# abcouwer-jpl/zsc

Measured on AMD Instinct MI355X. Metric: deflate level-6 uncompressed MB/s in, Canterbury-like x4096 per GPU, higher is better.
Workload: dtype u8

## Files before the change

__graft_entry__.py:

```python
from __future__ import annotations

import os
import subprocess
import sys

ROOT = os.path.dirname(os.path.abspath(__file__))
if ROOT not in sys.path:
    sys.path.insert(0, ROOT)


def build() -> None:
    subprocess.run(["make", "-s", "-C", os.path.join(ROOT, "zsc_amd", "csrc")], check=True)
    subprocess.run(["make", "-s", "-C", os.path.join(ROOT, "oracle"), "oracle", "ref"], check=True)
    subprocess.run(["make", "-s", "-C", os.path.join(ROOT, "tests", "emu")], check=True)
    subprocess.run(["make", "-s", "-C", os.path.join(ROOT, "tests", "emu_sections")], check=True)
    subprocess.run(["make", "-s", "-C", os.path.join(ROOT, "tests", "emu_chunks")], check=True)
    subprocess.run(["make", "-s", "-C", os.path.join(ROOT, "tests", "emu_resync")], check=True)
    subprocess.run(["make", "-s", "-C", os.path.join(ROOT, "tests", "c_caller")], check=True)
    import zsc_amd


def smoke() -> None:
    import zsc_amd
    from zsc_amd import corpus
    from oracle.oracle_py import Oracle

    print("device:", zsc_amd.device_info())
    oracle = Oracle()
    bufs = [corpus.make_buffer(kind, size, 7 + i) for i, (kind, size) in enumerate(
        [("text", 70000), ("bitmap", 40000), ("table", 20000), ("random", 5000), ("zero", 3000),
         ("token", 257), ("text", 0)])]
    rc, outs, stats = zsc_amd.compress_batch(bufs, level=6)
# ... 18 lines not shown
```

include/zsc_hip.h:

```cpp
#ifndef ZSC_HIP_H
#define ZSC_HIP_H

#include <stdint.h>

#include "zsc/zlib_types_pub.h"

#ifdef __cplusplus
extern "C" {
#endif


I32 zsc_hip_init(I32 device_ordinal);

const char *zsc_hip_device_info(void);

void zsc_hip_release_cached_memory(void);


ZlibReturn zsc_hip_compress_batch(U32 count, const U8 *const *sources, const U32 *source_lens,
                                  U8 *const *dests, U32 *dest_lens, I32 *statuses, I32 level,
                                  I32 window_bits, I32 mem_level, ZlibStrategy strategy);

ZlibReturn zsc_hip_store_batch(U32 count, const U8 *const *sources, const U32 *source_lens,
                               const U32 *max_block_lens, U8 *const *dests, U32 *dest_lens,
// ... 32 lines not shown

ZlibReturn zsc_hip_deflate_plan_run(zsc_hip_deflate_plan *plan, const void *d_input,
                                    void *d_output, void *hip_stream);

ZlibReturn zsc_hip_deflate_plan_results(zsc_hip_deflate_plan *plan, U32 *dest_lens,
                                        I32 *statuses);

#define ZSC_HIP_NKERNELS 9
void zsc_hip_deflate_plan_profile(zsc_hip_deflate_plan *plan, I32 enable);
ZlibReturn zsc_hip_deflate_plan_times(zsc_hip_deflate_plan *plan, float *ms_out);

uint64_t zsc_hip_deflate_plan_scratch_bytes(const zsc_hip_deflate_plan *plan);

U32 zsc_hip_deflate_plan_sub_batches(const zsc_hip_deflate_plan *plan);

void zsc_hip_deflate_plan_destroy(zsc_hip_deflate_plan *plan);


typedef struct zsc_hip_inflate_plan zsc_hip_inflate_plan;

ZlibReturn zsc_hip_inflate_plan_create(zsc_hip_inflate_plan **plan, U32 count,
                                       const U32 *source_lens, const uint64_t *src_offsets,
                                       const U32 *dest_caps, const uint64_t *dst_offsets,
                                       I32 window_bits);
ZlibReturn zsc_hip_inflate_plan_create_ordered(zsc_hip_inflate_plan **plan, U32 count,
                                               const U32 *source_lens, const uint64_t *src_offsets,
                                               const U32 *dest_caps, const uint64_t *dst_offsets,
                                               I32 window_bits, const U32 *decode_order);
ZlibReturn zsc_hip_inflate_plan_run(zsc_hip_inflate_plan *plan, const void *d_src, void *d_dst,
                                    void *hip_stream);
// ... 37 lines not shown
```

zsc_amd/api.py:

```python
from __future__ import annotations

import ctypes as C
import os
import subprocess
from typing import List, Optional, Sequence, Tuple

Z_OK, Z_STREAM_END, Z_NEED_DICT = 0, 1, 2
Z_ERRNO, Z_STREAM_ERROR, Z_DATA_ERROR, Z_MEM_ERROR, Z_BUF_ERROR, Z_VERSION_ERROR = -1, -2, -3, -4, -5, -6
Z_DEFAULT_STRATEGY, Z_FILTERED, Z_HUFFMAN_ONLY, Z_RLE, Z_FIXED = 0, 1, 2, 3, 4
GZIP_CODE, DEF_WBITS, DEF_MEM_LEVEL = 16, 15, 8
NKERNELS = 9
KERNEL_NAMES = ("checksum", "hash_sort", "match_table", "parse", "parse_short", "huff_plan", "layout", "emit", "total")

_HERE = os.path.dirname(os.path.abspath(__file__))
lib_path = os.environ.get("ZSC_HIP_LIB") or os.path.join(_HERE, "libzsc_hip.so")


def build_library() -> None:
    subprocess.run(["make", "-s", "-C", os.path.join(_HERE, "csrc")], check=True)


def _load() -> C.CDLL:
    try:
        import torch
# ... 50 lines not shown
    L.zsc_hip_inflate_plan_destroy.argtypes = [C.c_void_p]
    L.zsc_hip_inflate_plan_destroy.restype = None
    L.zsc_hip_deflate_plan_layout.argtypes = [C.c_uint32, u32p, C.c_int32, C.c_int32, C.c_int32,
                                              u64p, u64p, u32p, u64p, u64p]
    L.zsc_hip_deflate_plan_create.argtypes = [C.POINTER(C.c_void_p), C.c_uint32, u32p, u64p, u64p,
                                              u32p, C.c_int32, C.c_int32, C.c_int32, C.c_int32]
    L.zsc_hip_deflate_plan_run.argtypes = [C.c_void_p, C.c_void_p, C.c_void_p, C.c_void_p]
    L.zsc_hip_deflate_plan_results.argtypes = [C.c_void_p, u32p, i32p]
    L.zsc_hip_deflate_plan_profile.argtypes = [C.c_void_p, C.c_int32]
    L.zsc_hip_deflate_plan_profile.restype = None
    L.zsc_hip_deflate_plan_times.argtypes = [C.c_void_p, C.POINTER(C.c_float)]
    L.zsc_hip_deflate_plan_scratch_bytes.argtypes = [C.c_void_p]
    L.zsc_hip_deflate_plan_scratch_bytes.restype = C.c_uint64
    L.zsc_hip_deflate_plan_sub_batches.argtypes = [C.c_void_p]
    L.zsc_hip_deflate_plan_sub_batches.restype = C.c_uint32
    L.zsc_hip_deflate_plan_destroy.argtypes = [C.c_void_p]
    L.zsc_hip_deflate_plan_destroy.restype = None
    return L


lib = _load()


def device_info() -> str:
    return lib.zsc_hip_device_info().decode()



def compress_get_min_work_buf_size(window_bits: int = DEF_WBITS, mem_level: int = DEF_MEM_LEVEL):
    out = C.c_uint32()
# ... 324 lines not shown
        self.out_caps = list(self._caps)
        self._h = C.c_void_p()
        rc = lib.zsc_hip_deflate_plan_create(C.byref(self._h), n, lens, self._in_off, self._out_off,
                                             self._caps, level, window_bits, mem_level, strategy)
        if rc != Z_OK:
            raise RuntimeError(f"zsc_hip_deflate_plan_create failed: {rc}")

    @property
    def scratch_bytes(self) -> int:
        return lib.zsc_hip_deflate_plan_scratch_bytes(self._h)

    @property
    def sub_batches(self) -> int:
        return lib.zsc_hip_deflate_plan_sub_batches(self._h)

    def profile(self, enable: bool = True) -> None:
        lib.zsc_hip_deflate_plan_profile(self._h, 1 if enable else 0)

    def run(self, d_input: int, d_output: int, stream: int = 0) -> None:
        rc = lib.zsc_hip_deflate_plan_run(self._h, C.c_void_p(d_input), C.c_void_p(d_output),
                                          C.c_void_p(stream))
        if rc != Z_OK:
            raise RuntimeError(f"zsc_hip_deflate_plan_run failed: {rc}")

    def results(self) -> Tuple[List[int], List[int]]:
        lens = (C.c_uint32 * self.count)()
        stat = (C.c_int32 * self.count)()
        rc = lib.zsc_hip_deflate_plan_results(self._h, lens, stat)
        if rc != Z_OK:
            raise RuntimeError(f"zsc_hip_deflate_plan_results failed: {rc}")
# ... 20 lines not shown
```

zsc_amd/csrc/lz_parse.h:

```cpp
#ifndef ZSC_LZ_PARSE_H
#define ZSC_LZ_PARSE_H

#include "wave.h"
#include "zsc_dev.h"

#define LZ_PR 512u
#define LZ_MIRROR 512u
#define LZ_PR_FAST 128u

template <uint32_t RING_BYTES, uint32_t CHUNK_BYTES, bool WITH_HOLES = false>
struct LzLdsT {
    static constexpr uint32_t RING = RING_BYTES, CHUNK = CHUNK_BYTES;
    static constexpr bool HAS_INS = WITH_HOLES;
    static constexpr bool HOLES = WITH_HOLES;
    static constexpr bool GLOBAL_WIN = false;
    static constexpr uint32_t PR = LZ_PR;
    uint8_t ring[RING + 512];
    uint32_t stage[WAVE];
    uint16_t prank[LZ_PR];
    uint16_t phib[LZ_PR];
    uint32_t ins[WITH_HOLES ? RING / 32 : 1];
};
typedef LzLdsT<ZD_RING, ZD_CHUNK> LzLds;
typedef LzLdsT<18432u, 2048u> LzLds16k;
// ... 53 lines not shown
} LzJob;

typedef struct {
    uint32_t lo, hi;
    uint32_t wrap_base;
    uint32_t base;
    uint32_t data_end;
    uint32_t nsyms, nstaged;
    uint32_t nblocks, blk_sym0, blk_in0;
    uint32_t pr_hi;
    uint32_t n;
    uint32_t si;
    uint32_t it;
} LzState;

template <class L>
DEV uint32_t lz_ridx(const LzState &st, uint32_t pos)
{
    uint32_t r = pos - st.wrap_base;
    return r >= L::RING ? r - L::RING : r;
}

template <class L>
DEV uint32_t lz_w32(const LzJob &job, const L *lds, const LzState &st, uint32_t pos)
{
    if constexpr (L::GLOBAL_WIN) {
        (void)lds;
        (void)st;
        if ((uint64_t)pos + 4u <= job.ntot)
            return ld_u32(job.in + pos);
        uint32_t v = 0;
        for (uint32_t k = 0; k < 4u; k++)
            v |= (pos + k < job.ntot ? (uint32_t)job.in[pos + k] : 0u) << (8u * k);
// ... 759 lines not shown
```

zsc_amd/csrc/lz_parse_seg.h:

```cpp
#ifndef ZSC_LZ_PARSE_SEG_H
#define ZSC_LZ_PARSE_SEG_H

#include "lz_parse.h"

#ifdef SG_GROUP
#undef ZSC_GROUP
#define ZSC_GROUP SG_GROUP
#include "wave_group.h"
#endif

#ifndef SG_COUNT
#define SG_COUNT(what, n)
#endif

#ifndef SG_W
#define SG_W 8
#endif
#ifndef SG_G
#define SG_G 256u
#endif
#ifndef SG_SPAN
#define SG_SPAN 8192u
#endif
#ifndef SG_MIN_WAVES
// ... 53 lines not shown
    static constexpr bool HAS_INS = false;
    static constexpr bool GLOBAL_WIN = false;
    uint8_t ring[RING + 512];
    uint32_t trace[SG_NS][SG_TRACE / 32];
    uint32_t tkind[SG_NS][SG_TRACE / 32];
    SgWave wv[SG_NS];
    uint32_t S0;
    uint32_t finished;
    uint32_t queue;
    uint32_t redo, redo_seg, redo_from;
    uint32_t chain, chain_ft;
    uint32_t emu_ascending;
    uint32_t lo, hi, wrap_base;
    SgOut out;
    uint32_t cstage[WAVE];
};

typedef struct {
    uint32_t *tok;
    uint16_t *sidx;
} SgScratch;

DEV uint32_t sg_base_at(const ZdLevel &cfg, uint32_t p, uint32_t n, uint32_t need)
{
    uint32_t base = 0;
    for (;;) {
        uint64_t end = (uint64_t)base + 2ull * cfg.wsize;
        uint32_t data_end = end < n ? (uint32_t)end : n;
        if ((uint64_t)p + need > data_end && p - base >= cfg.wsize + cfg.max_dist)
            base += cfg.wsize;
// ... 50 lines not shown
    {
        lds->lo = st.lo;
        lds->hi = st.hi;
        lds->wrap_base = st.wrap_base;
        lds->queue = sg_nact(S0, job.n);
        lds->redo = 0;
        lds->chain = 0;
        lds->chain_ft = 0;
    }
    FOR_LANES
    {
        for (uint32_t i = (uint32_t)LANE; i < SG_NS * (SG_TRACE / 32); i += WAVE)
            (&lds->trace[0][0])[i] = 0;
    }
    WAVE_SYNC();
}


#define SG_PEEK32(pos, out) ((out) = GUNI(lds_u32(lds->ring, lz_ridx<L>(st, (pos)))))
#define SG_PEEKP(OFF, out) ((out) = GUNI(lds_u32(lds->ring, rp + (OFF))))

#define SG_LOAD(E, B)                                                                         \
    FOR_GLANES                                                                                 \
    {                                                                                         \
        const uint32_t _v = (B)*GRP + (uint32_t)GLANE;                                         \
        int32_t _i = _v < nA ? hiA - (int32_t)_v : hiB - (int32_t)(_v - nA) - (int32_t)ZD_TILE; \
        _i = _v < total ? _i : 0;                                                             \
        LV(E) = job.sorted[(uint32_t)((int32_t)tileA + _i)];  \
    }

// ... 444 lines not shown
    do {                                                                                      \
        LANEVAR(int, _fr);                                                                    \
        LANEVAR(int, _kd);                                                                    \
        FOR_GLANES                                                                             \
        {                                                                                     \
            sidx[sd_blk * GRP + (uint32_t)GLANE] = (uint16_t)LV(sdx);                          \
            LV(_fr) = (int)((LV(sdx) >> 16) & 1u);                                            \
            LV(_kd) = (int)((LV(sdx) >> 17) & 1u);                                            \
        }                                                                                     \
        const uint64_t _mf = GBALLOT(_fr), _mk = GBALLOT(_kd);                                  \
        ON_GLANE0                                                                              \
        {                                                                                     \
            if (GRP >= 32u) {                                                                 \
                for (uint32_t _j = 0; _j < GRP / 32u; _j++) {                                 \
                    const uint32_t _w = sd_blk * (GRP / 32u) + _j;                            \
                    lds->tkind[s][_w] = (uint32_t)(_mk >> (32u * _j));                        \
                    LDS_STORE_REL(&lds->trace[s][_w], (uint32_t)(_mf >> (32u * _j)));         \
                }                                                                             \
            } else {  \
                const uint32_t _w = sd_blk * GRP / 32u, _sh = sd_blk * GRP % 32u;             \
                const uint32_t _m = ((1u << (GRP & 31u)) - 1u) << _sh;                        \
                lds->tkind[s][_w] = (lds->tkind[s][_w] & ~_m) | ((uint32_t)_mk << _sh);       \
                LDS_STORE_REL(&lds->trace[s][_w], (lds->trace[s][_w] & ~_m) | ((uint32_t)_mf << _sh)); \
            }                                                                                 \
        }                                                                                     \
    } while (0)

#define SG_EMIT(SYM)                                                                          \
    do {                                                                                      \
        const uint32_t _sym = (SYM);                                                          \
        FOR_GLANES                                                                             \
        {                                                                                     \
            if ((uint32_t)GLANE == nstaged)                                                    \
                LV(stg) = _sym;                                                               \
        }                                                                                     \
        nstaged++;                                                                            \
        ntok++;                                                                               \
        if (nstaged == GRP) {                                                                 \
            FOR_GLANES { tok[ntok - GRP + (uint32_t)GLANE] = LV(stg); }                        \
            nstaged = 0;                                                                      \
        }                                                                                     \
    } while (0)

template <bool TABLE>
DEV void sg_parse_segment(const LzJob &job, SgLds *lds, const SgScratch &scr, uint32_t s,
                          uint32_t p, uint32_t cur_len, uint32_t cur_at, int pending)
{
    typedef SgLds L;
    LzState st;
    st.lo = GUNI(lds->lo);
    st.hi = GUNI(lds->hi);
    st.wrap_base = GUNI(lds->wrap_base);
    st.nsyms = st.nstaged = st.nblocks = st.blk_sym0 = st.blk_in0 = st.pr_hi = 0;
    st.n = job.n;
    st.si = 0;
    st.it = 0;

    const uint32_t S0 = GUNI(lds->S0);
    const uint64_t E64 = (uint64_t)S0 + SG_SPAN;
    const uint32_t E = E64 < job.n ? (uint32_t)E64 : job.n;
    const uint32_t a_s = S0 + s * SG_G;
    const uint32_t e_s = a_s + SG_G < E ? a_s + SG_G : E;

    st.base = sg_base(job.cfg, p, job.n);
    {
        uint64_t end = (uint64_t)st.base + 2ull * job.cfg.wsize;
        st.data_end = end < job.n ? (uint32_t)end : job.n;
    }
    uint32_t *tok = scr.tok + s * SG_TOKCAP;
    uint16_t *sidx = scr.sidx + s * SG_TRACE;
    uint32_t ntok = 0, nstaged = 0, exit_kind = 0;

    LANEVAR(uint32_t, mha);
    LANEVAR(uint32_t, mhb);
    LANEVAR(uint32_t, mna);
    LANEVAR(uint32_t, mto);
    LANEVAR(uint32_t, mfl);
    LANEVAR(uint32_t, mhf);
    LANEVAR(uint32_t, mby);
    LANEVAR(uint32_t, mcp);
    LANEVAR(uint32_t, mni);
    LANEVAR(uint32_t, pv);
    LANEVAR(uint32_t, stg);
    LANEVAR(uint32_t, sdx);
    LANEVAR(uint32_t, hop);
// ... 11 lines not shown
        uint32_t look = st.data_end - p;
        if (look < ZD_MIN_LOOKAHEAD) {
            const uint32_t base0 = st.base, end0 = st.data_end;
            lz_refill(job, st, p);
            if (st.base != base0 || st.data_end != end0)
                mt_at = p + 4096u;
            look = st.data_end - p;
            if (look == 0) {
                exit_kind = SG_EXIT_END;
                break;
            }
        }
        SG_COUNT(4, 1);
        const int fresh = cur_len == 2u;
        if (p >= e_s) {
            if (p >= E) {
                exit_kind = SG_EXIT_LAST;
                break;
            }
            if (fresh) {
                const uint32_t t = (p - S0) / SG_G, r = (p - S0) % SG_G;
                const uint32_t tword = GUNI(LDS_LOAD_ACQ(&lds->trace[t][r >> 5]));
                if (((tword >> (r & 31u)) & 1u) &&
                    ((GUNI(lds->tkind[t][r >> 5]) >> (r & 31u)) & 1u) == (uint32_t)pending) {
                    exit_kind = SG_EXIT_SYNCED;
                    break;
                }
            }
            if (p >= e_s + SG_OV) {
                exit_kind = SG_EXIT_UNSYNCED;
                break;
            }
        } else if (fresh) {
            const uint32_t r = p - a_s;
            if (r / GRP != sd_blk) {
                if (sd_blk != 0xffffffffu)
                    SG_TRACE_FLUSH();
                sd_blk = r / GRP;
                FOR_GLANES { LV(sdx) = 0; }
// ... 428 lines not shown
            p++;
        }
        lit = s0123 & 0xffu;
        if (emit)
            SG_EMIT(sym);
    }
    FOR_GLANES
    {
        if ((uint32_t)GLANE < nstaged)
            tok[ntok - nstaged + (uint32_t)GLANE] = LV(stg);
    }
    if (sd_blk != 0xffffffffu)
        SG_TRACE_FLUSH();
    ON_GLANE0
    {
        SgWave *me = &lds->wv[s];
        me->exit_kind = exit_kind;
        me->exit_p = p;
        me->exit_len = cur_len;
        me->exit_at = cur_at;
        me->exit_pending = (uint32_t)pending;
        me->ntok = ntok;
    }
    WAVE_SYNC();
}

template <bool TABLE>
DEV void sg_phase_parse(const LzJob &job, SgLds *lds, const SgScratch &scr, int w)
{
    const uint32_t S0 = GUNI(lds->S0);
    const uint32_t nact = sg_nact(S0, job.n);
// ... 99 lines not shown
            blk_sym0 = nsyms;
            blk_in0 = cov;
        }
    }
    ON_LANE0
    {
        o->nsyms = nsyms;
        o->nblocks = nblocks;
        o->blk_sym0 = blk_sym0;
        o->blk_in0 = blk_in0;
        o->cov = cov;
    }
    WAVE_SYNC();
}

DEV void sg_phase_resolve(const LzJob &job, SgLds *lds, const SgScratch &scr, int w)
{
    if (w != 0)
        return;
    const uint32_t S0 = UNI(lds->S0);
    uint32_t k = UNI(lds->chain), ft = UNI(lds->chain_ft);
    for (;;) {
        const uint32_t kind = UNI(lds->wv[k].exit_kind);
        const uint32_t xp = UNI(lds->wv[k].exit_p);
        sg_append(job, &lds->out, scr.tok + k * SG_TOKCAP, ft, UNI(lds->wv[k].ntok), 1, 1u, ZD_MIN_LOOKAHEAD);
        if (kind == SG_EXIT_SYNCED) {
            const uint32_t t = (xp - S0) / SG_G;
            ft = UNI(scr.sidx[t * SG_TRACE + (xp - S0) % SG_G]);
            k = t;
            continue;
// ... 11 lines not shown
            return;
        }
        if (kind == SG_EXIT_LAST) {
            ON_LANE0
            {
                lds->wv[0].start_p = xp;
                lds->wv[0].start_len = lds->wv[k].exit_len;
                lds->wv[0].start_at = lds->wv[k].exit_at;
                lds->wv[0].start_pending = lds->wv[k].exit_pending;
                lds->S0 += SG_SPAN;
                lds->redo = 0;
            }
            WAVE_SYNC();
            return;
        }
        if (UNI(lds->wv[k].exit_pending)) {
            const uint32_t c = UNI(job.in[xp - 1]);
            ON_LANE0 { lds->cstage[0] = c; }
            WAVE_SYNC();
            sg_append(job, &lds->out, lds->cstage, 0, 1, 0, 1u, ZD_MIN_LOOKAHEAD);
        }
        ON_LANE0
        {
            const uint32_t cutting = !job.more || lds->out.nsyms != lds->out.blk_sym0;
            if (cutting) {
                ZdBlockRec *b = &job.blocks[lds->out.nblocks];
                b->sym_begin = lds->out.blk_sym0;
                b->sym_count = lds->out.nsyms - lds->out.blk_sym0;
                b->in_begin = lds->out.blk_in0;
                b->in_len = job.n - lds->out.blk_in0;
                b->stored_ok = lds->out.blk_in0 >= sg_base(job.cfg, job.n, job.n) ? 1u : 0u;
                b->last = job.more ? 0u : 1u;
                b->cut = ZD_CUT_END;
                b->wend = 0xffffffffu;
                b->at = job.n;
                lds->out.nblocks++;
                lds->out.blk_sym0 = lds->out.nsyms;
                lds->out.blk_in0 = job.n;
            }
            job.out->nsyms = lds->out.nsyms;
            job.out->nblocks = lds->out.nblocks;
            lds->redo = 0;
            lds->finished = 1;
        }
        WAVE_SYNC();
        return;
    }
}

DEV void sg_next_phase(SgLds *lds, int w, uint32_t from)
{
    if (w != 0)
        return;
    ON_LANE0
    {
        lds->S0 = from;
// ... 53 lines not shown
```

zsc_amd/csrc/wave.h:

```cpp
#ifndef ZSC_WAVE_H
#define ZSC_WAVE_H

#include <stdint.h>

#ifndef WAVE
#define WAVE 64
#endif

#ifdef ZSC_WAVE_EMU
#include <string.h>

#define DEV static inline
#define DEV_OUTLINED static
#define GLOBAL_FN static
#define LDS_DECL(T, name, n) T name[n]
#define LANEVAR(T, name) T name[WAVE]
#define LV(name) name[_lane]
#define UNROLL_FULL
#define LANEARR(T, name, n) T name[n][WAVE]
#define LVA(name, k) name[k][_lane]
#define LV_UNIFORM(name) name[0]
#define FOR_LANES for (int _lane = 0; _lane < WAVE; ++_lane)
#define LANE (_lane)
#define ON_LANE0
// ... 54 lines not shown
{
    uint16_t v;
    memcpy(&v, p, 2);
    return v;
}
static inline uint32_t lds_u32(const uint8_t *base, uint32_t idx)
{
    return ld_u32(base + idx);
}
#define LDS_ADD_U32(ptr, v) (*(ptr) += (v))
#define LDS_FETCH_ADD_U32(ptr, v) ((*(ptr) += (v)) - (v))
#define LDS_OR_U32(ptr, v) (*(ptr) |= (v))
#define GLOBAL_OR_U32(ptr, v) (*(ptr) |= (v))
#define LDS_STORE_REL(ptr, v) (*(ptr) = (v))
#define LDS_LOAD_ACQ(ptr) (*(ptr))
#define CTZ64(x) __builtin_ctzll(x)
#define CTZ32(x) __builtin_ctz(x)
#define POPC64(x) __builtin_popcountll(x)
#define CLZ64(x) __builtin_clzll(x)
#define CLZ32(x) __builtin_clz(x)
static inline uint32_t emu_brev32(uint32_t v)
{
    v = ((v >> 1) & 0x55555555u) | ((v & 0x55555555u) << 1);
    v = ((v >> 2) & 0x33333333u) | ((v & 0x33333333u) << 2);
    v = ((v >> 4) & 0x0f0f0f0fu) | ((v & 0x0f0f0f0fu) << 4);
    v = ((v >> 8) & 0x00ff00ffu) | ((v & 0x00ff00ffu) << 8);
    return (v >> 16) | (v << 16);
}
#define BREV32(x) emu_brev32(x)
#define COPY16(dst, src) memcpy((dst), (src), 16)
// ... 82 lines not shown
    uint16_t v;
    __builtin_memcpy(&v, p, 2);
    return v;
}
DEV uint32_t lds_u32(const uint8_t *base, uint32_t idx)
{
    const uint32_t *w = (const uint32_t *)(base + (idx & ~3u));
    return __builtin_amdgcn_alignbyte(w[1], w[0], idx & 3u);
}
#define LDS_ADD_U32(ptr, v) atomicAdd((ptr), (v))
#define LDS_FETCH_ADD_U32(ptr, v) atomicAdd((ptr), (v))
#define LDS_OR_U32(ptr, v) atomicOr((ptr), (v))
#define GLOBAL_OR_U32(ptr, v) atomicOr((ptr), (v))
#define LDS_STORE_REL(ptr, v) __hip_atomic_store((ptr), (v), __ATOMIC_RELEASE, __HIP_MEMORY_SCOPE_WORKGROUP)
#define LDS_LOAD_ACQ(ptr) __hip_atomic_load((ptr), __ATOMIC_ACQUIRE, __HIP_MEMORY_SCOPE_WORKGROUP)
#define CTZ64(x) __builtin_ctzll(x)
#define CTZ32(x) __builtin_ctz(x)
#define POPC64(x) __builtin_popcountll(x)
#define CLZ64(x) __builtin_clzll(x)
#define CLZ32(x) __builtin_clz(x)
#define BREV32(x) __builtin_bitreverse32(x)
#define UNI(x) ((uint32_t)__builtin_amdgcn_readfirstlane((int)(x)))
#define OPAQUE_UNI(x) asm volatile("" : "+s"(x))
#define COPY16(dst, src) (*(uint4 *)(dst) = *(const uint4 *)(src))
#define RCP_F32(x) __builtin_amdgcn_rcpf(x)

#endif

#include "wave_group.h"

// ... 2 lines not shown
```

zsc_amd/csrc/zsc_hip_runtime.hip:

```cpp
#include <hip/hip_runtime.h>

#include <algorithm>
#include <chrono>
#include <cstdio>
#include <cstdlib>
#include <cstring>
#include <mutex>
#include <vector>

#include "bit_emit.h"
#include "checksum.h"
#include "hash_sort.h"
#include "huff_plan.h"
#include "inflate.h"
#include "inflate_sections.h"
#include "inflate_chunks.h"
#include "inflate_resync.h"
#include "lz_parse.h"
#include "lz_parse_seg.h"
#include "match_table.h"
#include "lz_parse_simple.h"
#include "sections.h"
#include "zsc_dev.h"

#include "zsc/zsc_conf_private.h"
#include "zsc_hip.h"


__global__ __launch_bounds__(64) void k_checksum(const uint8_t *__restrict__ in,
                                                 const ZdBuf *__restrict__ bufs,
                                                 ZdResult *__restrict__ res, uint32_t nbuf)
{
    __shared__ CkLds lds;
    const uint32_t b = blockIdx.x;
// ... 234 lines not shown
__global__ __launch_bounds__(SG_W * 64, SG_MIN_WAVES) void k_parse_seg(const uint8_t *__restrict__ in,
                                                         const ZdBuf *__restrict__ bufs,
                                                         const uint32_t *__restrict__ order,
                                                         const uint32_t *__restrict__ sorted,
                                                         const uint16_t *__restrict__ rank,
                                                         const uint16_t *__restrict__ hib,
                                                         const uint32_t *__restrict__ cnt,
                                                         const uint16_t *__restrict__ dir,
                                                         const uint32_t *__restrict__ r2,
                                                         uint32_t *__restrict__ syms,
                                                         ZdBlockRec *__restrict__ recs,
                                                         ZdParseOut *__restrict__ pout,
                                                         uint32_t *__restrict__ seg_tok,
                                                         const ZdSched *__restrict__ sched,
                                                         const ZdLevel cfg, uint32_t stair_min,
                                                         uint32_t first, uint32_t nbuf)
{
    __shared__ SgLds lds;
    if (blockIdx.x >= nbuf)
        return;
    const uint32_t b = order[first + blockIdx.x];
    const ZdBuf buf = bufs[b];
    LzJob job;
    job.in = in + buf.in_off;
    job.n = buf.in_len;
    job.ntot = buf.in_len;
    job.sorted = sorted + (uint64_t)buf.tile0 * ZD_TILE;
    job.rank = rank + buf.rank_off;
    job.hib = hib + buf.rank_off;
    job.cnt = cnt + buf.rank_off;
    job.dir = dir ? dir + (uint64_t)buf.tile0 * ZD_DIR_STRIDE : nullptr;
// ... 13 lines not shown
        job.cfg.good = 8;
        job.cfg.lazy = 16;
        job.cfg.nice = 128;
        job.cfg.chain = 128;
        job.cfg.slow = 1;
    }
    job.strategy = LEVEL == 6 ? 0u : buf.strategy;
    job.more = buf.more;
    job.sched = sched + buf.sched_off;
    job.nsched = buf.sched_n;
    job.n0 = buf.n0;
    SgScratch scr;
    scr.tok = seg_tok + (uint64_t)blockIdx.x * SG_SCRATCH_WORDS;
    scr.sidx = (uint16_t *)(scr.tok + SG_NS * SG_TOKCAP);
    const int w = (int)(threadIdx.x >> 6);
    sg_init(&lds, w);
    __syncthreads();
    const uint32_t max_steps = buf.in_len / SG_SPAN + 2;
    bool stuck = false;
    uint32_t si = 0, nph = buf.sched_n ? buf.n0 : buf.in_len;
    for (uint32_t phase = 0; phase <= buf.sched_n && !stuck; phase++) {
        nph = sg_phase_end(job, nph, &si);
        const bool goes_on = si < buf.sched_n;
        job.n = nph;
        job.more = goes_on ? 1u : buf.more;
        uint32_t steps = 0;
        while (!lds.finished) {
            if (++steps > max_steps) {
                stuck = true;
                break;
// ... 574 lines not shown
struct zsc_hip_deflate_plan {
    uint32_t count = 0;
    int level = 6, wrap = 1, wbits = 15, mem_level = 8;
    uint32_t strategy = 0;
    std::vector<ZdBuf> bufs;
    std::vector<SubBatch> subs;
    DevBuf d_sorted, d_tmp_syms, d_rank, d_hib, d_cnt, d_dir, d_recs, d_plans, d_pout;
    DevBuf d_seg_tok;
    DevBuf d_r2;
    bool use_table = false;
    uint32_t table_min = 0;
    uint32_t table_cap = MT_CAP;
    uint32_t stair_min = SG_STAIR_MIN;
    DevBuf d_sched;
    bool use_seg = true;
    DevBuf d_res;
    uint64_t rank_base_off = 0;
    bool profile = false;
    float times[ZSC_HIP_NKERNELS] = {0};
    std::vector<hipEvent_t> events;
    size_t events_used = 0;
    uint32_t profiled_runs = 0;
    hipStream_t last_stream = nullptr;
    uint64_t scratch_bytes = 0;
};

namespace {
void ensure_init()
{
    int before = -1;
// ... 199 lines not shown
            sb.nslots += b.max_blocks;
            sb.nsym_slots += ((uint64_t)n + 64u) & ~63ull;
            bytes += n;
            sb.count++;
            i++;
        }
        max_tiles = std::max<uint64_t>(max_tiles, sb.ntiles);
        max_slots = std::max<uint64_t>(max_slots, sb.nslots);
        max_syms = std::max<uint64_t>(max_syms, sb.nsym_slots);
        max_rank_span = std::max<uint64_t>(max_rank_span, sb.nsym_slots + 64);
        max_count = std::max<uint64_t>(max_count, sb.count);
        pl->subs.push_back(std::move(sb));
    }

    pl->use_seg = getenv("ZSC_HIP_NO_SEG") == nullptr && kLevels[level].slow;
    for (SubBatch &sb : pl->subs) {
        std::vector<uint32_t> tile_owner(sb.ntiles), blk_owner(sb.nslots), order(sb.count);
        for (uint32_t k = 0; k < sb.count; k++) {
            const ZdBuf &b = pl->bufs[sb.first + k];
            for (uint32_t t = 0; t < b.ntiles; t++)
                tile_owner[b.tile0 + t] = k;
            for (uint32_t s = 0; s < b.max_blocks; s++)
                blk_owner[b.blk0 + s] = k;
            order[k] = k;
        }
        static const uint32_t seg_min = getenv("ZSC_HIP_SEG_MIN") ? (uint32_t)atoi(getenv("ZSC_HIP_SEG_MIN")) : 3072u;
        pl->table_min = seg_min;
        auto seg_able = [&](uint32_t k) {
            const ZdBuf &b = pl->bufs[sb.first + k];
            return pl->use_seg && b.in_len > seg_min && (b.sched_n == 0 || b.seg_ok);
// ... 141 lines not shown
        uint32_t *sorted = (uint32_t *)pl->d_sorted.p;
        uint32_t *tmp_syms = (uint32_t *)pl->d_tmp_syms.p;
        uint16_t *rank = (uint16_t *)pl->d_rank.p;
        uint16_t *hib = (uint16_t *)pl->d_hib.p;
        uint32_t *cnt = (uint32_t *)pl->d_cnt.p;
        uint16_t *dir = (uint16_t *)pl->d_dir.p;
        ZdBlockRec *recs = (ZdBlockRec *)pl->d_recs.p;
        ZdBlockPlan *plans = (ZdBlockPlan *)pl->d_plans.p;
        ZdParseOut *pout = (ZdParseOut *)pl->d_pout.p;

        mark();
        hipLaunchKernelGGL(k_checksum, dim3(sb.count), dim3(64), 0, st, in, bufs, res, sb.count);
        mark();
        const bool simple = pl->strategy == (uint32_t)Z_HUFFMAN_ONLY || pl->strategy == (uint32_t)Z_RLE;
        const bool link_in_parser = !simple && cfg.slow && sb.cseg == sb.count && !pl->use_table &&
                                    getenv("ZSC_HIP_LINK_KERNEL") == nullptr;
        if (!simple) {
            hipLaunchKernelGGL(k_hash_sort, dim3(sb.ntiles), dim3(HS_WAVES * 64), 0, st, in, bufs,
                               (const uint32_t *)sb.d_tile_owner.p, sorted, tmp_syms, rank, dir,
                               sb.ntiles);
            if (!link_in_parser)
                hipLaunchKernelGGL(k_link_prev, dim3(sb.ntiles), dim3(HS_WAVES * 64), 0, st, in, bufs,
                                   (const uint32_t *)sb.d_tile_owner.p, (const uint16_t *)dir,
                                   (const uint16_t *)rank, hib, cnt, sb.ntiles);
        }
        mark();
        if (!simple) {
            if (pl->use_table && sb.cseg > 0)
                hipLaunchKernelGGL(k_match_table, dim3(sb.ntiles), dim3(MT_WAVES * 64), 0, st, in, bufs,
                                   (const uint32_t *)sb.d_tile_owner.p, (const uint32_t *)sorted,
                                   (const uint16_t *)rank, (const uint16_t *)hib, (const uint32_t *)cnt,
// ... 12 lines not shown
                       (const uint32_t *)sb.d_order.p, (const uint32_t *)sorted,                 \
                       (const uint16_t *)rank, (const uint16_t *)hib, tmp_syms, recs, pout,      \
                       (const ZdSched *)pl->d_sched.p, cfg, (uint32_t)(FIRST), (uint32_t)(COUNT))
            if (sb.cseg > 0) {
                auto kern = (pl->wbits == 15 && pl->mem_level == 8)
                                ? (pl->use_table ? k_parse_seg<false, true, 0>
                                                 : pl->level == 6 && pl->strategy != (uint32_t)Z_FILTERED ? k_parse_seg<false, false, 6>
                                                                                                          : k_parse_seg<false, false, 0>)
                                : k_parse_seg<true, false, 0>;
                hipLaunchKernelGGL(kern, dim3(sb.cseg), dim3(SG_W * 64), 0, st, in, bufs,
                                   (const uint32_t *)sb.d_order.p, (const uint32_t *)sorted,
                                   (const uint16_t *)rank, (const uint16_t *)hib,
                                   (const uint32_t *)cnt, link_in_parser ? (const uint16_t *)dir : nullptr,
                                   pl->use_table ? (const uint32_t *)pl->d_r2.p : nullptr, tmp_syms, recs,
                                   pout, (uint32_t *)pl->d_seg_tok.p,
                                   (const ZdSched *)pl->d_sched.p, cfg, pl->stair_min, 0u, sb.cseg);
            }
            if (pl->d_sched.p) {
                ZSC_LAUNCH_PARSE(LzLdsJ, sb.cseg, sb.c36 - sb.cseg);
                mark();
                ZSC_LAUNCH_PARSE(LzLdsJ16k, sb.c36, sb.c16 - sb.c36);
                ZSC_LAUNCH_PARSE(LzLdsJ8k, sb.c16, sb.c8 - sb.c16);
                ZSC_LAUNCH_PARSE(LzLdsJ4k, sb.c8, sb.count - sb.c8);
            } else {
                ZSC_LAUNCH_PARSE(LzLds, sb.cseg, sb.c36 - sb.cseg);
                mark();
                ZSC_LAUNCH_PARSE(LzLds16k, sb.c36, sb.c16 - sb.c36);
                ZSC_LAUNCH_PARSE(LzLds8k, sb.c16, sb.c8 - sb.c16);
                ZSC_LAUNCH_PARSE(LzLds4k, sb.c8, sb.count - sb.c8);
            }
#undef ZSC_LAUNCH_PARSE
        } else
            hipLaunchKernelGGL(getenv("ZSC_HIP_FAST_RING") ? k_parse_fast<LzLdsFast> : k_parse_fast<LzLdsFastG>,
                               dim3(sb.count), dim3(64), 0, st, in, bufs,
                               (const uint32_t *)sb.d_order.p, (const uint32_t *)sorted,
                               (const uint16_t *)rank, (const uint16_t *)hib, tmp_syms, recs,
                               pout, (const ZdSched *)pl->d_sched.p, cfg, sb.count);
        if (!simple && !cfg.slow)
            mark();
        mark();
        hipLaunchKernelGGL(k_huff_plan, dim3(sb.nslots), dim3(64), 0, st, bufs,
                           (const uint32_t *)sb.d_blk_owner.p, (const uint32_t *)tmp_syms,
                           (const ZdBlockRec *)recs, (const ZdParseOut *)pout, plans, sb.nslots);
        mark();
        hipLaunchKernelGGL(k_layout, dim3((sb.count + 63) / 64), dim3(64), 0, st, bufs,
                           (const ZdParseOut *)pout, (const ZdBlockRec *)recs, plans, res, out,
                           sb.count);
        mark();
// ... 55 lines not shown
    ZSC_ASSERT(pl != Z_NULL);
    ZSC_ASSERT(ms_out != Z_NULL);
    for (int k = 0; k < ZSC_HIP_NKERNELS; k++)
        ms_out[k] = pl->times[k];
    return pl->profile ? Z_OK : Z_STREAM_ERROR;
}

extern "C" uint64_t zsc_hip_deflate_plan_scratch_bytes(const zsc_hip_deflate_plan *pl)
{
    return pl ? pl->scratch_bytes : 0;
}

extern "C" U32 zsc_hip_deflate_plan_sub_batches(const zsc_hip_deflate_plan *pl)
{
    return pl ? (U32)pl->subs.size() : 0;
}

extern "C" void zsc_hip_deflate_plan_destroy(zsc_hip_deflate_plan *pl)
{
    DeviceScope scope;
    if (!pl)
        return;
    (void)hipStreamSynchronize(pl->last_stream);
    for (SubBatch &sb : pl->subs) {
        sb.d_bufs.release();
        sb.d_tile_owner.release();
        sb.d_blk_owner.release();
        sb.d_order.release();
    }
    pl->d_sorted.release();
// ... 1436 lines not shown
```

Before: 6697.

## Replace segmented-parse super-steps with a work-stealing pipeline across waves

Adds a pipelined schedule for the segmented LZ parser. Waves in a workgroup claim jobs (redo, resolve, chunk load, segment parse) through LDS compare-and-swap flags instead of moving in lock-step super-steps, and the segment slots are reused as a ring of SG_NS entries. The goal is to overlap input loading, parsing and chain resolution and to remove barrier idle time between phases. In exchange it adds atomic and spin traffic, sleep-based waiting, and a stuck-detection fallback that marks the output invalid. Host getenv calls are also cached at plan creation.

```diff
diff --git a/__graft_entry__.py b/__graft_entry__.py
--- a/__graft_entry__.py
+++ b/__graft_entry__.py
@@ -16,6 +16,7 @@
     subprocess.run(["make", "-s", "-C", os.path.join(ROOT, "tests", "emu_sections")], check=True)
     subprocess.run(["make", "-s", "-C", os.path.join(ROOT, "tests", "emu_chunks")], check=True)
     subprocess.run(["make", "-s", "-C", os.path.join(ROOT, "tests", "emu_resync")], check=True)
+    subprocess.run(["make", "-s", "-C", os.path.join(ROOT, "tests", "emu_pipe")], check=True)
     subprocess.run(["make", "-s", "-C", os.path.join(ROOT, "tests", "c_caller")], check=True)
     import zsc_amd
 
diff --git a/include/zsc_hip.h b/include/zsc_hip.h
--- a/include/zsc_hip.h
+++ b/include/zsc_hip.h
@@ -70,6 +70,8 @@
 
 U32 zsc_hip_deflate_plan_sub_batches(const zsc_hip_deflate_plan *plan);
 
+I32 zsc_hip_deflate_plan_seg_schedule(const zsc_hip_deflate_plan *plan);
+
 void zsc_hip_deflate_plan_destroy(zsc_hip_deflate_plan *plan);
 
 
diff --git a/zsc_amd/api.py b/zsc_amd/api.py
--- a/zsc_amd/api.py
+++ b/zsc_amd/api.py
@@ -88,6 +88,8 @@
     L.zsc_hip_deflate_plan_scratch_bytes.restype = C.c_uint64
     L.zsc_hip_deflate_plan_sub_batches.argtypes = [C.c_void_p]
     L.zsc_hip_deflate_plan_sub_batches.restype = C.c_uint32
+    L.zsc_hip_deflate_plan_seg_schedule.argtypes = [C.c_void_p]
+    L.zsc_hip_deflate_plan_seg_schedule.restype = C.c_int32
     L.zsc_hip_deflate_plan_destroy.argtypes = [C.c_void_p]
     L.zsc_hip_deflate_plan_destroy.restype = None
     return L
@@ -442,6 +444,10 @@
     def sub_batches(self) -> int:
         return lib.zsc_hip_deflate_plan_sub_batches(self._h)
 
+    @property
+    def seg_schedule(self) -> str:
+        return ("none", "super-steps", "pipeline")[lib.zsc_hip_deflate_plan_seg_schedule(self._h)]
+
     def profile(self, enable: bool = True) -> None:
         lib.zsc_hip_deflate_plan_profile(self._h, 1 if enable else 0)
 
diff --git a/zsc_amd/csrc/lz_parse.h b/zsc_amd/csrc/lz_parse.h
--- a/zsc_amd/csrc/lz_parse.h
+++ b/zsc_amd/csrc/lz_parse.h
@@ -91,9 +91,13 @@
     uint32_t it;
 } LzState;
 
+#ifndef LZ_RING_HOOK
+#define LZ_RING_HOOK(st, pos)
+#endif
 template <class L>
 DEV uint32_t lz_ridx(const LzState &st, uint32_t pos)
 {
+    LZ_RING_HOOK(st, pos);
     uint32_t r = pos - st.wrap_base;
     return r >= L::RING ? r - L::RING : r;
 }
diff --git a/zsc_amd/csrc/lz_parse_pipe.h b/zsc_amd/csrc/lz_parse_pipe.h
--- /dev/null
+++ b/zsc_amd/csrc/lz_parse_pipe.h
@@ -0,0 +1,249 @@
+#ifndef ZSC_LZ_PARSE_PIPE_H
+#define ZSC_LZ_PARSE_PIPE_H
+
+#include "lz_parse_seg.h"
+
+#ifndef SG_PIPE_HOOK_LOAD
+#define SG_PIPE_HOOK_LOAD(hi, released)
+#endif
+
+#define SG_PIPE_DONE 0
+#define SG_PIPE_WORKED 1
+#define SG_PIPE_IDLE 2
+
+#define SG_JOB_REDO 1u
+#define SG_JOB_RESOLVE 2u
+#define SG_JOB_LOAD 4u
+#define SG_JOB_PARSE 8u
+#define SG_JOB_ALL 15u
+
+#define SG_PIPE_NOXP 0xffffffffu
+
+DEV uint32_t sg_pipe_floor(uint32_t released)
+{
+    const uint32_t a = released * SG_G;
+    return a > ZD_TILE ? a - ZD_TILE : 0u;
+}
+DEV bool sg_pipe_may_load(uint32_t hi, uint32_t released)
+{
+    return (uint64_t)hi + SgLds::CHUNK <= (uint64_t)SgLds::RING + sg_pipe_floor(released);
+}
+DEV uint32_t sg_pipe_want(uint32_t g, uint32_t ntot)
+{
+    const uint64_t e = ((uint64_t)g + 1u) * SG_G + SG_OV + 2u * ZD_MIN_LOOKAHEAD;
+    return e < ntot ? (uint32_t)e : ntot;
+}
+DEV uint32_t sg_pipe_nseg(uint32_t n)
+{
+    return n == 0 ? 1u : (uint32_t)(((uint64_t)n + SG_G - 1u) / SG_G);
+}
+
+DEV bool sg_pipe_claim(uint32_t *word, uint32_t from, uint32_t to)
+{
+    LANEVAR(uint32_t, got);
+    FOR_LANES
+    {
+        LV(got) = 0;
+        if (LANE == 0)
+            LV(got) = LDS_CAS_U32(word, from, to);
+    }
+    return READLANE(got, 0) == from;
+}
+
+DEV void sg_pipe_init(SgLds *lds, int w)
+{
+    sg_init(lds, w);
+    if (w != 0)
+        return;
+    FOR_LANES
+    {
+        for (uint32_t i = (uint32_t)LANE; i < SG_NS * (SG_TRACE / 32); i += WAVE)
+            (&lds->trace[0][0])[i] = 0;
+        for (uint32_t i = (uint32_t)LANE; i < SG_NS; i += WAVE)
+            lds->p_done[i] = 0;
+    }
+    ON_LANE0
+    {
+        lds->p_next = 0;
+        lds->p_released = 0;
+        lds->p_res_busy = lds->p_load_busy = 0;
+        lds->p_redo = 0;
+        lds->p_rs[0] = lds->p_rs[1] = lds->p_rs[2] = lds->p_rs[3] = 0;
+        lds->p_chain_xp = SG_PIPE_NOXP;
+        lds->p_stuck = 0;
+    }
+    WAVE_SYNC();
+}
+
+DEV void sg_pipe_resolve(const LzJob &job, SgLds *lds, const SgScratch &scr)
+{
+    if (UNI(LDS_LOAD_ACQ(&lds->finished)) != 0u)
+        return;
+    const bool held = UNI(LDS_LOAD_ACQ(&lds->p_redo)) != 0u;
+    uint32_t k = UNI(lds->chain), ft = UNI(lds->chain_ft), cxp = UNI(lds->p_chain_xp);
+    uint32_t rel = UNI(lds->p_released);
+    for (;;) {
+        const uint32_t rel0 = rel;
+        while (rel < k && UNI(LDS_LOAD_ACQ(&lds->p_done[rel % SG_NS])) == rel + 1u) {
+            FOR_LANES
+            {
+                if ((uint32_t)LANE < SG_TRACE / 32)
+                    lds->trace[rel % SG_NS][LANE] = 0;
+            }
+            rel++;
+        }
+        if (rel != rel0) {
+            WAVE_SYNC();
+            ON_LANE0 { LDS_STORE_REL(&lds->p_released, rel); }
+        }
+        const uint32_t ks = k % SG_NS;
+        if (held)
+            return;
+        if (UNI(LDS_LOAD_ACQ(&lds->p_done[ks])) != k + 1u)
+            break;
+        if (cxp != SG_PIPE_NOXP) {
+            ft = UNI(scr.sidx[ks * SG_TRACE + cxp % SG_G]);
+            cxp = SG_PIPE_NOXP;
+        }
+        const uint32_t kind = UNI(lds->wv[ks].exit_kind);
+        const uint32_t xp = UNI(lds->wv[ks].exit_p);
+        sg_append(job, &lds->out, scr.tok + ks * SG_TOKCAP, ft, UNI(lds->wv[ks].ntok), 1, 1u, ZD_MIN_LOOKAHEAD);
+        if (kind == SG_EXIT_SYNCED) {
+            k = xp / SG_G;
+            cxp = xp;
+            ft = 0;
+            continue;
+        }
+        if (kind == SG_EXIT_UNSYNCED || kind == SG_EXIT_LAST) {
+            const uint32_t xl = UNI(lds->wv[ks].exit_len), xa = UNI(lds->wv[ks].exit_at);
+            const uint32_t xn = UNI(lds->wv[ks].exit_pending);
+            k = xp / SG_G;
+            ft = 0;
+            ON_LANE0
+            {
+                lds->p_rs[0] = xp;
+                lds->p_rs[1] = xl;
+                lds->p_rs[2] = xa;
+                lds->p_rs[3] = xn;
+                lds->redo_seg = k;
+                lds->chain = k;
+                lds->chain_ft = 0;
+                lds->p_chain_xp = SG_PIPE_NOXP;
+                LDS_STORE_REL(&lds->p_redo, 1u);
+            }
+            WAVE_SYNC();
+            return;
+        }
+        sg_end_of_input(job, lds, UNI(lds->wv[ks].exit_pending), xp);
+        ON_LANE0 { LDS_STORE_REL(&lds->finished, 1u); }
+        WAVE_SYNC();
+        return;
+    }
+    ON_LANE0
+    {
+        lds->chain = k;
+        lds->chain_ft = ft;
+        lds->p_chain_xp = cxp;
+    }
+    WAVE_SYNC();
+}
+
+template <bool TABLE>
+DEV int sg_pipe_step(const LzJob &job, SgLds *lds, const SgScratch &scr, uint32_t allow)
+{
+    if (UNI(LDS_LOAD_ACQ(&lds->finished)) != 0u)
+        return SG_PIPE_DONE;
+    const uint32_t redo = UNI(LDS_LOAD_ACQ(&lds->p_redo));
+    if ((allow & SG_JOB_REDO) && redo == 1u) {
+        const uint32_t t = UNI(lds->redo_seg);
+        if (UNI(LDS_LOAD_ACQ(&lds->p_done[t % SG_NS])) == t + 1u && sg_pipe_claim(&lds->p_redo, 1u, 2u)) {
+            const uint32_t sp = UNI(lds->p_rs[0]), sl = UNI(lds->p_rs[1]), sa = UNI(lds->p_rs[2]);
+            const uint32_t sn = UNI(lds->p_rs[3]);
+            SG_COUNT(2, 0x10000 + t);
+            sg_parse_segment<TABLE, true>(job, lds, scr, t, sp, sl, sa, (int)sn);
+            SG_COUNT(3, 0);
+            ON_LANE0 { LDS_STORE_REL(&lds->p_redo, 0u); }
+            return SG_PIPE_WORKED;
+        }
+    }
+    const uint32_t rel = UNI(LDS_LOAD_ACQ(&lds->p_released));
+    if ((allow & SG_JOB_RESOLVE) && UNI(LDS_LOAD_ACQ(&lds->p_res_busy)) == 0u) {
+        const uint32_t k = UNI(LDS_LOAD_ACQ(&lds->chain));
+        if (((redo == 0u && UNI(LDS_LOAD_ACQ(&lds->p_done[k % SG_NS])) == k + 1u) ||
+             (rel < k && UNI(LDS_LOAD_ACQ(&lds->p_done[rel % SG_NS])) == rel + 1u)) &&
+            sg_pipe_claim(&lds->p_res_busy, 0u, 1u)) {
+            sg_pipe_resolve(job, lds, scr);
+            ON_LANE0 { LDS_STORE_REL(&lds->p_res_busy, 0u); }
+            return SG_PIPE_WORKED;
+        }
+    }
+    uint32_t hi = UNI(LDS_LOAD_ACQ(&lds->hi));
+    if ((allow & SG_JOB_LOAD) && hi < job.ntot && sg_pipe_may_load(hi, rel) &&
+        UNI(LDS_LOAD_ACQ(&lds->p_load_busy)) == 0u && sg_pipe_claim(&lds->p_load_busy, 0u, 1u)) {
+        hi = UNI(LDS_LOAD_ACQ(&lds->hi));
+        if (hi < job.ntot && sg_pipe_may_load(hi, rel)) {
+            SG_PIPE_HOOK_LOAD(hi, rel);
+            LzState st;
+            st.hi = hi;
+            st.lo = 0;
+            st.wrap_base = hi / SgLds::RING * SgLds::RING;
+            lz_load_chunk<SgLds>(job, lds, st);
+            ON_LANE0 { LDS_STORE_REL(&lds->hi, st.hi); }
+        }
+        ON_LANE0 { LDS_STORE_REL(&lds->p_load_busy, 0u); }
+        return SG_PIPE_WORKED;
+    }
+    if (allow & SG_JOB_PARSE) {
+        const uint32_t g = UNI(LDS_LOAD_ACQ(&lds->p_next));
+        if (g < sg_pipe_nseg(job.n) && g < rel + SG_NS && hi >= sg_pipe_want(g, job.ntot) &&
+            sg_pipe_claim(&lds->p_next, g, g + 1u)) {
+            SG_COUNT(2, g);
+            sg_parse_segment<TABLE, true>(job, lds, scr, g, g * SG_G, 2u, 0u, 0);
+            SG_COUNT(3, 0);
+            ON_LANE0 { LDS_STORE_REL(&lds->p_done[g % SG_NS], g + 1u); }
+            return SG_PIPE_WORKED;
+        }
+    }
+    return SG_PIPE_IDLE;
+}
+
+#ifndef ZSC_WAVE_EMU
+DEV uint32_t sg_pipe_progress(SgLds *lds)
+{
+    return UNI(LDS_LOAD_ACQ(&lds->p_next)) + UNI(LDS_LOAD_ACQ(&lds->p_released)) + UNI(LDS_LOAD_ACQ(&lds->hi)) +
+           UNI(LDS_LOAD_ACQ(&lds->chain)) + UNI(LDS_LOAD_ACQ(&lds->p_redo));
+}
+
+#define SG_PIPE_MAX_IDLE (1u << 20)
+
+template <bool TABLE>
+DEV void sg_pipe_run(const LzJob &job, SgLds *lds, const SgScratch &scr)
+{
+    uint32_t idle = 0, row = 0, seen = 0;
+    for (;;) {
+        const int r = sg_pipe_step<TABLE>(job, lds, scr, SG_JOB_ALL);
+        if (r == SG_PIPE_DONE)
+            break;
+        if (r == SG_PIPE_WORKED) {
+            row = idle = 0;
+            continue;
+        }
+        const uint32_t now = sg_pipe_progress(lds);
+        if (now != seen) {
+            seen = now;
+            idle = 0;
+        }
+        if (++idle > SG_PIPE_MAX_IDLE) {
+            ON_LANE0
+            {
+                lds->p_stuck = 1;
+                LDS_STORE_REL(&lds->finished, 1u);
+            }
+            break;
+        }
+        WAVE_NAP(++row > 8u);
+    }
+}
+#endif
+
+#endif
diff --git a/zsc_amd/csrc/lz_parse_seg.h b/zsc_amd/csrc/lz_parse_seg.h
--- a/zsc_amd/csrc/lz_parse_seg.h
+++ b/zsc_amd/csrc/lz_parse_seg.h
@@ -91,6 +91,14 @@
     uint32_t lo, hi, wrap_base;
     SgOut out;
     uint32_t cstage[WAVE];
+    uint32_t p_done[SG_NS];
+    uint32_t p_next;
+    uint32_t p_released;
+    uint32_t p_res_busy, p_load_busy;
+    uint32_t p_redo;
+    uint32_t p_rs[4];
+    uint32_t p_chain_xp;
+    uint32_t p_stuck;
 };
 
 typedef struct {
@@ -171,6 +179,16 @@
             (&lds->trace[0][0])[i] = 0;
     }
     WAVE_SYNC();
+}
+
+DEV uint32_t sg_pipe_wrap_base(uint32_t p)
+{
+    return p > ZD_TILE ? (p - ZD_TILE) / SgLds::RING * SgLds::RING : 0u;
+}
+DEV uint32_t sg_pipe_limit(SgLds *lds, uint32_t n)
+{
+    const uint64_t e = ((uint64_t)GUNI(LDS_LOAD_ACQ(&lds->p_released)) + SG_NS) * SG_G;
+    return e < n ? (uint32_t)e : n;
 }
 
 
@@ -645,14 +663,14 @@
             if (GRP >= 32u) {                                                                 \
                 for (uint32_t _j = 0; _j < GRP / 32u; _j++) {                                 \
                     const uint32_t _w = sd_blk * (GRP / 32u) + _j;                            \
-                    lds->tkind[s][_w] = (uint32_t)(_mk >> (32u * _j));                        \
-                    LDS_STORE_REL(&lds->trace[s][_w], (uint32_t)(_mf >> (32u * _j)));         \
+                    lds->tkind[slot][_w] = (uint32_t)(_mk >> (32u * _j));                        \
+                    LDS_STORE_REL(&lds->trace[slot][_w], (uint32_t)(_mf >> (32u * _j)));         \
                 }                                                                             \
             } else {  \
                 const uint32_t _w = sd_blk * GRP / 32u, _sh = sd_blk * GRP % 32u;             \
                 const uint32_t _m = ((1u << (GRP & 31u)) - 1u) << _sh;                        \
-                lds->tkind[s][_w] = (lds->tkind[s][_w] & ~_m) | ((uint32_t)_mk << _sh);       \
-                LDS_STORE_REL(&lds->trace[s][_w], (lds->trace[s][_w] & ~_m) | ((uint32_t)_mf << _sh)); \
+                lds->tkind[slot][_w] = (lds->tkind[slot][_w] & ~_m) | ((uint32_t)_mk << _sh);       \
+                LDS_STORE_REL(&lds->trace[slot][_w], (lds->trace[slot][_w] & ~_m) | ((uint32_t)_mf << _sh)); \
             }                                                                                 \
         }                                                                                     \
     } while (0)
@@ -673,7 +691,7 @@
         }                                                                                     \
     } while (0)
 
-template <bool TABLE>
+template <bool TABLE, bool PIPE = false>
 DEV void sg_parse_segment(const LzJob &job, SgLds *lds, const SgScratch &scr, uint32_t s,
                           uint32_t p, uint32_t cur_len, uint32_t cur_at, int pending)
 {
@@ -681,15 +699,16 @@
     LzState st;
     st.lo = GUNI(lds->lo);
     st.hi = GUNI(lds->hi);
-    st.wrap_base = GUNI(lds->wrap_base);
+    st.wrap_base = PIPE ? sg_pipe_wrap_base(p) : GUNI(lds->wrap_base);
     st.nsyms = st.nstaged = st.nblocks = st.blk_sym0 = st.blk_in0 = st.pr_hi = 0;
     st.n = job.n;
     st.si = 0;
     st.it = 0;
 
-    const uint32_t S0 = GUNI(lds->S0);
+    const uint32_t slot = PIPE ? s % SG_NS : s;
+    const uint32_t S0 = PIPE ? 0u : GUNI(lds->S0);
     const uint64_t E64 = (uint64_t)S0 + SG_SPAN;
-    const uint32_t E = E64 < job.n ? (uint32_t)E64 : job.n;
+    uint32_t E = PIPE ? job.n : E64 < job.n ? (uint32_t)E64 : job.n;
     const uint32_t a_s = S0 + s * SG_G;
     const uint32_t e_s = a_s + SG_G < E ? a_s + SG_G : E;
 
@@ -698,8 +717,8 @@
         uint64_t end = (uint64_t)st.base + 2ull * job.cfg.wsize;
         st.data_end = end < job.n ? (uint32_t)end : job.n;
     }
-    uint32_t *tok = scr.tok + s * SG_TOKCAP;
-    uint16_t *sidx = scr.sidx + s * SG_TRACE;
+    uint32_t *tok = scr.tok + slot * SG_TOKCAP;
+    uint16_t *sidx = scr.sidx + slot * SG_TRACE;
     uint32_t ntok = 0, nstaged = 0, exit_kind = 0;
 
     LANEVAR(uint32_t, mha);
@@ -741,15 +760,18 @@
         SG_COUNT(4, 1);
         const int fresh = cur_len == 2u;
         if (p >= e_s) {
+            if (PIPE)
+                E = sg_pipe_limit(lds, job.n);
             if (p >= E) {
                 exit_kind = SG_EXIT_LAST;
                 break;
             }
             if (fresh) {
                 const uint32_t t = (p - S0) / SG_G, r = (p - S0) % SG_G;
-                const uint32_t tword = GUNI(LDS_LOAD_ACQ(&lds->trace[t][r >> 5]));
+                const uint32_t ts = PIPE ? t % SG_NS : t;
+                const uint32_t tword = GUNI(LDS_LOAD_ACQ(&lds->trace[ts][r >> 5]));
                 if (((tword >> (r & 31u)) & 1u) &&
-                    ((GUNI(lds->tkind[t][r >> 5]) >> (r & 31u)) & 1u) == (uint32_t)pending) {
+                    ((GUNI(lds->tkind[ts][r >> 5]) >> (r & 31u)) & 1u) == (uint32_t)pending) {
                     exit_kind = SG_EXIT_SYNCED;
                     break;
                 }
@@ -1208,7 +1230,7 @@
         SG_TRACE_FLUSH();
     ON_GLANE0
     {
-        SgWave *me = &lds->wv[s];
+        SgWave *me = &lds->wv[slot];
         me->exit_kind = exit_kind;
         me->exit_p = p;
         me->exit_len = cur_len;
@@ -1338,6 +1360,38 @@
     WAVE_SYNC();
 }
 
+DEV void sg_end_of_input(const LzJob &job, SgLds *lds, uint32_t pending, uint32_t xp)
+{
+    if (pending) {
+        const uint32_t c = UNI(job.in[xp - 1]);
+        ON_LANE0 { lds->cstage[0] = c; }
+        WAVE_SYNC();
+        sg_append(job, &lds->out, lds->cstage, 0, 1, 0, 1u, ZD_MIN_LOOKAHEAD);
+    }
+    ON_LANE0
+    {
+        const uint32_t cutting = !job.more || lds->out.nsyms != lds->out.blk_sym0;
+        if (cutting) {
+            ZdBlockRec *b = &job.blocks[lds->out.nblocks];
+            b->sym_begin = lds->out.blk_sym0;
+            b->sym_count = lds->out.nsyms - lds->out.blk_sym0;
+            b->in_begin = lds->out.blk_in0;
+            b->in_len = job.n - lds->out.blk_in0;
+            b->stored_ok = lds->out.blk_in0 >= sg_base(job.cfg, job.n, job.n) ? 1u : 0u;
+            b->last = job.more ? 0u : 1u;
+            b->cut = ZD_CUT_END;
+            b->wend = 0xffffffffu;
+            b->at = job.n;
+            lds->out.nblocks++;
+            lds->out.blk_sym0 = lds->out.nsyms;
+            lds->out.blk_in0 = job.n;
+        }
+        job.out->nsyms = lds->out.nsyms;
+        job.out->nblocks = lds->out.nblocks;
+    }
+    WAVE_SYNC();
+}
+
 DEV void sg_phase_resolve(const LzJob &job, SgLds *lds, const SgScratch &scr, int w)
 {
     if (w != 0)
@@ -1379,32 +1433,9 @@
             WAVE_SYNC();
             return;
         }
-        if (UNI(lds->wv[k].exit_pending)) {
-            const uint32_t c = UNI(job.in[xp - 1]);
-            ON_LANE0 { lds->cstage[0] = c; }
-            WAVE_SYNC();
-            sg_append(job, &lds->out, lds->cstage, 0, 1, 0, 1u, ZD_MIN_LOOKAHEAD);
-        }
+        sg_end_of_input(job, lds, UNI(lds->wv[k].exit_pending), xp);
         ON_LANE0
         {
-            const uint32_t cutting = !job.more || lds->out.nsyms != lds->out.blk_sym0;
-            if (cutting) {
-                ZdBlockRec *b = &job.blocks[lds->out.nblocks];
-                b->sym_begin = lds->out.blk_sym0;
-                b->sym_count = lds->out.nsyms - lds->out.blk_sym0;
-                b->in_begin = lds->out.blk_in0;
-                b->in_len = job.n - lds->out.blk_in0;
-                b->stored_ok = lds->out.blk_in0 >= sg_base(job.cfg, job.n, job.n) ? 1u : 0u;
-                b->last = job.more ? 0u : 1u;
-                b->cut = ZD_CUT_END;
-                b->wend = 0xffffffffu;
-                b->at = job.n;
-                lds->out.nblocks++;
-                lds->out.blk_sym0 = lds->out.nsyms;
-                lds->out.blk_in0 = job.n;
-            }
-            job.out->nsyms = lds->out.nsyms;
-            job.out->nblocks = lds->out.nblocks;
             lds->redo = 0;
             lds->finished = 1;
         }
diff --git a/zsc_amd/csrc/wave.h b/zsc_amd/csrc/wave.h
--- a/zsc_amd/csrc/wave.h
+++ b/zsc_amd/csrc/wave.h
@@ -92,6 +92,15 @@
 #define GLOBAL_OR_U32(ptr, v) (*(ptr) |= (v))
 #define LDS_STORE_REL(ptr, v) (*(ptr) = (v))
 #define LDS_LOAD_ACQ(ptr) (*(ptr))
+static inline uint32_t emu_lds_cas(uint32_t *p, uint32_t expect, uint32_t v)
+{
+    const uint32_t old = *p;
+    if (old == expect)
+        *p = v;
+    return old;
+}
+#define LDS_CAS_U32(ptr, expect, v) emu_lds_cas((ptr), (expect), (v))
+#define WAVE_NAP(long_one) ((void)0)
 #define CTZ64(x) __builtin_ctzll(x)
 #define CTZ32(x) __builtin_ctz(x)
 #define POPC64(x) __builtin_popcountll(x)
@@ -204,6 +213,13 @@
 #define GLOBAL_OR_U32(ptr, v) atomicOr((ptr), (v))
 #define LDS_STORE_REL(ptr, v) __hip_atomic_store((ptr), (v), __ATOMIC_RELEASE, __HIP_MEMORY_SCOPE_WORKGROUP)
 #define LDS_LOAD_ACQ(ptr) __hip_atomic_load((ptr), __ATOMIC_ACQUIRE, __HIP_MEMORY_SCOPE_WORKGROUP)
+DEV uint32_t lds_cas_u32(uint32_t *p, uint32_t expect, uint32_t v)
+{
+    __hip_atomic_compare_exchange_strong(p, &expect, v, __ATOMIC_ACQ_REL, __ATOMIC_ACQUIRE, __HIP_MEMORY_SCOPE_WORKGROUP);
+    return expect;
+}
+#define LDS_CAS_U32(ptr, expect, v) lds_cas_u32((ptr), (expect), (v))
+#define WAVE_NAP(long_one) ((long_one) ? __builtin_amdgcn_s_sleep(16) : __builtin_amdgcn_s_sleep(2))
 #define CTZ64(x) __builtin_ctzll(x)
 #define CTZ32(x) __builtin_ctz(x)
 #define POPC64(x) __builtin_popcountll(x)
diff --git a/zsc_amd/csrc/zsc_hip_runtime.hip b/zsc_amd/csrc/zsc_hip_runtime.hip
--- a/zsc_amd/csrc/zsc_hip_runtime.hip
+++ b/zsc_amd/csrc/zsc_hip_runtime.hip
@@ -18,6 +18,7 @@
 #include "inflate_resync.h"
 #include "lz_parse.h"
 #include "lz_parse_seg.h"
+#include "lz_parse_pipe.h"
 #include "match_table.h"
 #include "lz_parse_simple.h"
 #include "sections.h"
@@ -282,7 +283,7 @@
                                                          uint32_t *__restrict__ seg_tok,
                                                          const ZdSched *__restrict__ sched,
                                                          const ZdLevel cfg, uint32_t stair_min,
-                                                         uint32_t first, uint32_t nbuf)
+                                                         uint32_t pipe, uint32_t first, uint32_t nbuf)
 {
     __shared__ SgLds lds;
     if (blockIdx.x >= nbuf)
@@ -326,6 +327,20 @@
     scr.tok = seg_tok + (uint64_t)blockIdx.x * SG_SCRATCH_WORDS;
     scr.sidx = (uint16_t *)(scr.tok + SG_NS * SG_TOKCAP);
     const int w = (int)(threadIdx.x >> 6);
+    if (pipe && buf.sched_n == 0) {
+        sg_pipe_init(&lds, w);
+        __syncthreads();
+        if (TABLE && job.r2 != nullptr)
+            sg_pipe_run<true>(job, &lds, scr);
+        else
+            sg_pipe_run<false>(job, &lds, scr);
+        __syncthreads();
+        if (lds.p_stuck && threadIdx.x == 0) {
+            job.out->nsyms = 0;
+            job.out->nblocks = 0xffffffffu;
+        }
+        return;
+    }
     sg_init(&lds, w);
     __syncthreads();
     const uint32_t max_steps = buf.in_len / SG_SPAN + 2;
@@ -930,6 +945,9 @@
     uint32_t stair_min = SG_STAIR_MIN;
     DevBuf d_sched;
     bool use_seg = true;
+    bool seg_pipe = true;
+    bool link_kernel = false;
+    bool fast_ring = false;
     DevBuf d_res;
     uint64_t rank_base_off = 0;
     bool profile = false;
@@ -1159,6 +1177,10 @@
     }
 
     pl->use_seg = getenv("ZSC_HIP_NO_SEG") == nullptr && kLevels[level].slow;
+    if (const char *e = getenv("ZSC_HIP_SEG_PIPE"))
+        pl->seg_pipe = atoi(e) != 0;
+    pl->link_kernel = getenv("ZSC_HIP_LINK_KERNEL") != nullptr;
+    pl->fast_ring = getenv("ZSC_HIP_FAST_RING") != nullptr;
     for (SubBatch &sb : pl->subs) {
         std::vector<uint32_t> tile_owner(sb.ntiles), blk_owner(sb.nslots), order(sb.count);
         for (uint32_t k = 0; k < sb.count; k++) {
@@ -1330,7 +1352,7 @@
         mark();
         const bool simple = pl->strategy == (uint32_t)Z_HUFFMAN_ONLY || pl->strategy == (uint32_t)Z_RLE;
         const bool link_in_parser = !simple && cfg.slow && sb.cseg == sb.count && !pl->use_table &&
-                                    getenv("ZSC_HIP_LINK_KERNEL") == nullptr;
+                                    !pl->link_kernel;
         if (!simple) {
             hipLaunchKernelGGL(k_hash_sort, dim3(sb.ntiles), dim3(HS_WAVES * 64), 0, st, in, bufs,
                                (const uint32_t *)sb.d_tile_owner.p, sorted, tmp_syms, rank, dir,
@@ -1373,7 +1395,8 @@
                                    (const uint32_t *)cnt, link_in_parser ? (const uint16_t *)dir : nullptr,
                                    pl->use_table ? (const uint32_t *)pl->d_r2.p : nullptr, tmp_syms, recs,
                                    pout, (uint32_t *)pl->d_seg_tok.p,
-                                   (const ZdSched *)pl->d_sched.p, cfg, pl->stair_min, 0u, sb.cseg);
+                                   (const ZdSched *)pl->d_sched.p, cfg, pl->stair_min, pl->seg_pipe ? 1u : 0u, 0u,
+                                   sb.cseg);
             }
             if (pl->d_sched.p) {
                 ZSC_LAUNCH_PARSE(LzLdsJ, sb.cseg, sb.c36 - sb.cseg);
@@ -1390,7 +1413,7 @@
             }
 #undef ZSC_LAUNCH_PARSE
         } else
-            hipLaunchKernelGGL(getenv("ZSC_HIP_FAST_RING") ? k_parse_fast<LzLdsFast> : k_parse_fast<LzLdsFastG>,
+            hipLaunchKernelGGL(pl->fast_ring ? k_parse_fast<LzLdsFast> : k_parse_fast<LzLdsFastG>,
                                dim3(sb.count), dim3(64), 0, st, in, bufs,
                                (const uint32_t *)sb.d_order.p, (const uint32_t *)sorted,
                                (const uint16_t *)rank, (const uint16_t *)hib, tmp_syms, recs,
@@ -1476,6 +1499,13 @@
 extern "C" U32 zsc_hip_deflate_plan_sub_batches(const zsc_hip_deflate_plan *pl)
 {
     return pl ? (U32)pl->subs.size() : 0;
+}
+
+extern "C" I32 zsc_hip_deflate_plan_seg_schedule(const zsc_hip_deflate_plan *pl)
+{
+    if (!pl || !pl->use_seg)
+        return 0;
+    return pl->seg_pipe ? 2 : 1;
 }
 
 extern "C" void zsc_hip_deflate_plan_destroy(zsc_hip_deflate_plan *pl)
```

After: 7351 (median of 6 runs). +9.8%, better.
